# gk969/stm32-speech-recognition

Hardware: AMD Instinct MI355X
Metric: utterances/sec (256-frame, 100 templates) (higher is better)
Workload: dtype int32

## Files before the change

stm32_speech_recognition_amd/csrc/k_mfcc.hip:

```cpp
#include "sr_fft_dev.h"

#include <type_traits>

#ifndef SR_MEL_CHUNKED
#define SR_MEL_CHUNKED 1
#endif

namespace sr {

constexpr int kMfccWaves = 4;
constexpr int kFramesPerWave = 16, kFramesPerWaveMid = 4, kFramesPerWaveSmall = 1;
#ifndef SR_MAG_TAB_BINS
#define SR_MAG_TAB_BINS 8
#endif
constexpr int mfcc_tab_bins(int fpw) { return fpw == kFramesPerWave ? SR_MAG_TAB_BINS : 0; }
static_assert(SR_MAG_TAB_BINS == 0 || SR_MAG_TAB_BINS == 4 || SR_MAG_TAB_BINS == 8, "table bins per lane");
#ifndef SR_MFCC_PIPE
#define SR_MFCC_PIPE 1
#endif
#ifndef SR_MFCC_PIPE_PEEL
#define SR_MFCC_PIPE_PEEL 1
#endif
#ifndef SR_MFCC_PIPE_VMCNT
#define SR_MFCC_PIPE_VMCNT (SR_MFCC_PIPE_PEEL ? 3 : 0)
#endif
static_assert(SR_MFCC_PIPE_VMCNT == 0 || (SR_MFCC_PIPE_VMCNT == 3 && SR_MFCC_PIPE_PEEL), "younger loads counted by the wait");
constexpr bool mfcc_pipelined(int fpw) { return SR_MFCC_PIPE && mfcc_tab_bins(fpw) == 8; }
constexpr int kMelPad = kMel + 1;
__device__ __forceinline__ constexpr int mel_chunk_word(int j) { return 256 * ((j >> 2) & 1) + 4 * ((j >> 3) ^ (4 * ((j >> 2) & 1))) + (j & 3); }
constexpr int mfcc_wave_lds_words(int fpw) { return kXchgWords + fpw * kMelPad + 64; }

template <typename Base>
struct MfccTabArgs : Base {
    const uint16_t *mag_q;
    uint32_t mag_table_off;
};
template <typename Base>
constexpr int mfcc_feat_kind<MfccTabArgs<Base>> = mfcc_feat_kind<Base>;
template <typename Base>
static MfccTabArgs<Base> mfcc_tab_args(const Base &b, const MfccMagTab &tab)
{
    MfccTabArgs<Base> r;
    static_cast<Base &>(r) = b;
    r.mag_q = tab.mag_q;
    r.mag_table_off = tab.mag_table_off;
    return r;
}

template <int kFPW, typename Args = MfccTabArgs<MfccArgs>>
__global__ void __launch_bounds__(64 * kMfccWaves, 4) k_mfcc(const Args a)
{
    constexpr int kFeat = mfcc_feat_kind<Args>;
    constexpr uint32_t kFeatW = (kFeat == SR_FEAT_FFT || kFeat == SR_FEAT_MAG) ? kBins : kMel;
    constexpr int kWaveLdsWords = mfcc_wave_lds_words(kFPW);
    constexpr int kTabBins = mfcc_tab_bins(kFPW);
    constexpr bool kPipe = mfcc_pipelined(kFPW);
    extern __shared__ __attribute__((aligned(16))) uint32_t smem[];
    __shared__ uint32_t s_dctM[kCoef * kMelPad];
    __shared__ int s_dctS[kCoef * kMelPad];
    __shared__ u32x4 s_tw3[kTw3Row * 4], s_tw5[8 * 64];
    __shared__ u32x4 s_tm[4 * 64];
    const int lane = threadIdx.x & 63, w = __builtin_amdgcn_readfirstlane(threadIdx.x >> 6);
    uint32_t *buf = smem + w * kWaveLdsWords;
    uint32_t *xw = buf;
    uint32_t *powb = buf + kXchgWords, *moff = powb + kFPW * kMelPad;

    for (int i = threadIdx.x; i < kCoef * kMel; i += blockDim.x) {
        const int c = a.t.dct[i], o = (i / kMel) * kMelPad + i % kMel;
        s_dctM[o] = (uint32_t)(((c < 0 ? -c : c) * 262144 + 99) / 100);
        s_dctS[o] = (c > 0) - (c < 0);
    }
    __syncthreads();

    LaneTw tw;
    load_lane_tw(a.t, lane, tw);
    real_leg_tw(tw);
    if (w == 0 && lane < 4) {
        const uint32_t *f = &tw.s3[0][0][0];
#pragma unroll
        for (int c = 0; c < 8; c++) s_tw3[lane * kTw3Row + c] = u32x4{f[4 * c], f[4 * c + 1], f[4 * c + 2], f[4 * c + 3]};
    }
    if (w == 1 % kMfccWaves) store_tw32(s_tw5, lane, tw.s5);
#ifndef SR_INJECT_LDS_RACE
    if (w == 2 % kMfccWaves) {
#pragma unroll
        for (int c = 0; c < 2; c++) {
            s_tm[64 * c + lane] = *(const u32x4 *)(a.t.tri_even_m + 8 * lane + 4 * c);
            s_tm[64 * (c + 2) + lane] = *(const u32x4 *)(a.t.tri_odd_m + 8 * lane + 4 * c);
        }
    }
#endif
    __syncthreads();
#ifdef SR_INJECT_LDS_RACE
    if (w == 2 % kMfccWaves) {
#if SR_INJECT_LDS_RACE >= 2
        __builtin_amdgcn_s_sleep(127);
#endif
#pragma unroll
        for (int c = 0; c < 2; c++) {
            s_tm[64 * c + lane] = *(const u32x4 *)(a.t.tri_even_m + 8 * lane + 4 * c);
            s_tm[64 * (c + 2) + lane] = *(const u32x4 *)(a.t.tri_odd_m + 8 * lane + 4 * c);
        }
    }
#endif
    int hamm_m[3];
#pragma unroll
    for (int k = 0; k < 3; k++) hamm_m[k] = (lane + 64 * k < kFrameLen) ? hamm_fused_multiplier(a.t.hamm[lane + 64 * k]) : 0;
    int f_lo = 0, p_hi = 0, p_lo = 0, x_hi = 0, x_lo = 0;
    if (lane < kMel) {
        const int h = lane;
        f_lo = (h == 0) ? 0 : (int)a.t.tri_cen[h - 1];
        const int f_hi = (h == kMel - 1) ? kBins : (int)a.t.tri_cen[h + 1];
        const int ih = f_hi - 1, il = f_lo ? f_lo - 1 : 0, half = (h & 1) ? kBins : 0;
#if SR_MEL_CHUNKED
        p_hi = half + mel_chunk_word(ih), x_hi = (ih >> 3) > 0 ? (ih >> 3) - 1 : 0;
        p_lo = half + mel_chunk_word(il), x_lo = (il >> 3) > 0 ? (il >> 3) - 1 : 0;
#else
        p_hi = half + ih, x_hi = (ih >> 3) > 0 ? (ih >> 3) - 1 : 0;
        p_lo = half + il, x_lo = (il >> 3) > 0 ? (il >> 3) - 1 : 0;
#endif
    }
    const uint64_t mag_p = (uint64_t)a.mag_q;
    const u32x4 mag_rs = {(uint32_t)mag_p, (uint32_t)(mag_p >> 32) | (2u << 16), kMagTabEntries, 0x00027000u};
    const uint32_t tw_off = 32u * (uint32_t)lane;
#if SR_MEL_CHUNKED
    const int e_base = mel_chunk_word(lane);
    constexpr int kEs = 32, kEh = 128;
    const int c0 = mel_chunk_word(8 * lane), c1 = mel_chunk_word(8 * lane + 4);
#else
    const int e_base = lane;
    constexpr int kEs = 64, kEh = 256;
    const int c0 = 8 * lane, c1 = 8 * lane + 4;
#endif

    uint32_t item = blockIdx.x;
    uint32_t nx_nfrm = 0;
    int nx_mid = 0, nx_seg0 = 0;
    if (item < a.n_items) {
        const sr_vad_rec *rec = a.vad + item / a.tiles;
        nx_nfrm = rec->frm_num;
        nx_mid = (int)rec->atap.mid_val;
        nx_seg0 = rec->seg[0];
    }
    for (; item < a.n_items; item += gridDim.x) {
        const uint32_t b = item / a.tiles, tile = item - b * a.tiles;
        const uint32_t nfrm = nx_nfrm;
        const int mid = nx_mid, seg0 = nx_seg0;
        if (item + gridDim.x < a.n_items) {
            const sr_vad_rec *rec = a.vad + (item + gridDim.x) / a.tiles;
            nx_nfrm = rec->frm_num;
            nx_mid = (int)rec->atap.mid_val;
            nx_seg0 = rec->seg[0];
        }
        const uint16_t *row = a.pcm + (uint64_t)b * a.pcm_stride;
        int16_t *out = a.mfcc + (uint64_t)b * a.max_frames * kCoef;
        const uint32_t f0 = tile * (kMfccWaves * kFPW) + w * kFPW;
        uint32_t *frow = nullptr;
        if constexpr (kFeat != 0) frow = a.feat + (uint64_t)b * a.max_frames * kFeatW;
        uint32_t nf = 0;
        if (f0 < nfrm) nf = (nfrm - f0 < (uint32_t)kFPW) ? nfrm - f0 : (uint32_t)kFPW;

        uint32_t s_pp[3] = {0, 0, 0};
        if (nf) {
            const uint16_t *x = row + seg0 + (int)kHop * (int)f0;
#pragma unroll
            for (int k = 0; k < 3; k++) {
                const int i = lane + 64 * k;
                if (i < kFrameLen) s_pp[k] = *(const u32_align2 *)(x + i - 1);
            }
        }
        if constexpr (!kPipe)
        for (uint32_t fi = 0; fi < nf; fi++) {
#pragma unroll
            for (int k = 0; k < 3; k++) {
                const int i = lane + 64 * k;
                if (i < kFrameLen) k == 0 ? window_store<0>(xw, i, s_pp[k], mid, hamm_m[k]) : window_store<1>(xw, i, s_pp[k], mid, hamm_m[k]);
            }
            if (fi + 1 < nf) {
                const uint16_t *x = row + seg0 + (int)kHop * (int)(f0 + fi + 1);
#pragma unroll
                for (int k = 0; k < 3; k++) {
                    const int i = lane + 64 * k;
                    if (i < kFrameLen) s_pp[k] = *(const u32_align2 *)(x + i - 1);
                }
            }
            wave_sync();
            uint32_t v[4][4], u[4][4];
            fft_front_real160(xw, lane, tw, s_tw3, v);
            fft_exchange(buf, lane, v, u);
#pragma unroll
            for (int e4 = 0; e4 < 4; e4++) fft_pass4_dbl(u, e4, tw);
            wave_sync();
            uint32_t k5[4][4][2];
            load_tw32(s_tw5, lane, k5);
            uint32_t nn[8];
#pragma unroll
            for (int e3 = 0; e3 < 4; e3++) {
                bfly_pk_dbl<true, false, 0>(u[e3][0], u[e3][1], u[e3][2], u[e3][3], k5[e3][0][0], k5[e3][0][1], k5[e3][1][0],
                                            k5[e3][1][1], k5[e3][2][0], k5[e3][2][1], k5[e3][3][0], k5[e3][3][1]);
                if constexpr (kFeat == SR_FEAT_FFT) {
                    uint32_t *fr = frow + (f0 + fi) * kFeatW + lane + 64 * e3;
                    fr[0] = u[e3][0];
                    fr[256] = u[e3][1];
                }
                nn[2 * e3] = (uint32_t)sdot2z(u[e3][0], u[e3][0]);
                nn[2 * e3 + 1] = (uint32_t)sdot2z(u[e3][1], u[e3][1]);
            }
            const uint32_t nmax = max(max(max(max(nn[0], nn[1]), nn[2]), max(max(nn[3], nn[4]), nn[5])), max(nn[6], nn[7]));
#ifdef SR_TESTING
            const bool quiet = __builtin_expect(__builtin_amdgcn_ballot_w64(nmax > kMagSmallMax) == 0 && !a.mag_table_off, 1);
#else
            const bool quiet = __builtin_expect(__builtin_amdgcn_ballot_w64(nmax > kMagSmallMax) == 0, 1);
#endif
            u32x4 tw_e[2], tw_o[2];
            bool cheap = true;
            if (!quiet) {
#pragma unroll
                for (int c = 0; c < 2; c++) {
                    tw_e[c] = *(const u32x4 *)((const char *)a.t.tri_even32 + tw_off + 16 * c);
                    tw_o[c] = *(const u32x4 *)((const char *)a.t.tri_odd32 + tw_off + 16 * c);
                }
                cheap = __builtin_amdgcn_ballot_w64(nmax > a.mag_cheap_max) == 0;
            } else {
                asm volatile("" : "=v"(tw_e[0]), "=v"(tw_e[1]), "=v"(tw_o[0]), "=v"(tw_o[1]));
            }
            uint32_t *eb = buf + e_base;
            if (kTabBins > 0 && quiet) {
                uint32_t tq[8];
#pragma unroll
                for (int e3 = 0; e3 < 4; e3++) {
                    if constexpr (kTabBins == 8)
                        asm volatile("buffer_load_ushort %0, %1, %2, 0 idxen" : "=v"(tq[2 * e3]) : "v"(nn[2 * e3]), "s"(mag_rs));
                    asm volatile("buffer_load_ushort %0, %1, %2, 0 idxen" : "=v"(tq[2 * e3 + 1]) : "v"(nn[2 * e3 + 1]), "s"(mag_rs));
                }
                uint32_t q0s[4];
                if constexpr (kTabBins == 4) {
#pragma unroll
                    for (int e3 = 0; e3 < 4; e3++) q0s[e3] = cvt_u32(__builtin_amdgcn_sqrtf((float)(int)nn[2 * e3]) * 10.0f) << 2;
                }
                if constexpr (kTabBins == 8)
                    asm volatile("s_waitcnt vmcnt(0)" : "+v"(tq[0]), "+v"(tq[1]), "+v"(tq[2]), "+v"(tq[3]), "+v"(tq[4]), "+v"(tq[5]), "+v"(tq[6]), "+v"(tq[7]));
                else
                    asm volatile("s_waitcnt vmcnt(0)" : "+v"(tq[1]), "+v"(tq[3]), "+v"(tq[5]), "+v"(tq[7]));
#pragma unroll
                for (int e3 = 0; e3 < 4; e3++) {
                    uint32_t q0, q1 = tq[2 * e3 + 1];
                    if constexpr (kTabBins == 8) q0 = tq[2 * e3];
                    else q0 = q0s[e3];
                    if constexpr (kFeat == SR_FEAT_MAG) {
                        uint32_t *fr = frow + (f0 + fi) * kFeatW + lane + 64 * e3;
                        fr[0] = q0 >> 2;
                        fr[256] = q1 >> 2;
                    }
                    eb[kEs * e3] = umul24(q0, q0);
                    eb[kEs * e3 + kEh] = umul24(q1, q1);
                }
            } else if (cheap) {
#pragma unroll
                for (int e3 = 0; e3 < 4; e3++) {
                    const f32x2 m = f32x2{__builtin_amdgcn_sqrtf((float)(int)nn[2 * e3]), __builtin_amdgcn_sqrtf((float)(int)nn[2 * e3 + 1])} *
                                    f32x2{10.0f, 10.0f};
                    const uint32_t m0 = cvt_u32(m.x), m1 = cvt_u32(m.y);
                    if constexpr (kFeat == SR_FEAT_MAG) {
                        uint32_t *fr = frow + (f0 + fi) * kFeatW + lane + 64 * e3;
                        fr[0] = m0;
                        fr[256] = m1;
                    }
                    eb[kEs * e3] = umul24(m0, m0);
                    eb[kEs * e3 + kEh] = umul24(m1, m1);
                }
            } else {
#pragma unroll
                for (int e3 = 0; e3 < 4; e3++) {
                    const f32x2 m = sqrt_rn_int2(f32x2{(float)(int)nn[2 * e3], (float)(int)nn[2 * e3 + 1]}) * f32x2{10.0f, 10.0f};
                    const uint32_t m0 = cvt_u32(m.x), m1 = cvt_u32(m.y);
                    if constexpr (kFeat == SR_FEAT_MAG) {
                        uint32_t *fr = frow + (f0 + fi) * kFeatW + lane + 64 * e3;
                        fr[0] = m0;
                        fr[256] = m1;
                    }
                    eb[kEs * e3] = umul24(m0, m0);
                    eb[kEs * e3 + kEh] = umul24(m1, m1);
                }
            }
            wave_sync();
            uint32_t pe[8], po[8], xe, xo;
            {
                const uint4 q0 = *(const uint4 *)(buf + c0), q1 = *(const uint4 *)(buf + c1);
                const uint32_t e[8] = {q0.x, q0.y, q0.z, q0.w, q1.x, q1.y, q1.z, q1.w};
                uint32_t se = 0, so = 0;
                if (quiet) {
#pragma unroll
                    for (int c = 0; c < 2; c++) {
                        const u32x4 me = s_tm[64 * c + lane], mo = s_tm[64 * (c + 2) + lane];
#pragma unroll
                        for (int k = 0; k < 4; k++) {
                            const uint32_t es = kTabBins > 0 ? e[4 * c + k] : e[4 * c + k] << 4;
                            se += mel_term_fused(es, me[k]);
                            so += mel_term_fused(es, mo[k]);
                            pe[4 * c + k] = se;
                            po[4 * c + k] = so;
                        }
                    }
                } else {
#pragma unroll
                    for (int c = 0; c < 2; c++) {
#pragma unroll
                        for (int k = 0; k < 4; k++) {
                            se += e[4 * c + k] * tw_e[c][k] / 100u;
                            so += e[4 * c + k] * tw_o[c][k] / 100u;
                            pe[4 * c + k] = se;
                            po[4 * c + k] = so;
                        }
                    }
                }
                xe = wave_scan_incl(se);
                xo = wave_scan_incl(so);
            }
            *(uint4 *)(buf + c0) = make_uint4(pe[0], pe[1], pe[2], pe[3]);
            *(uint4 *)(buf + c1) = make_uint4(pe[4], pe[5], pe[6], pe[7]);
            *(uint4 *)(buf + kBins + c0) = make_uint4(po[0], po[1], po[2], po[3]);
            *(uint4 *)(buf + kBins + c1) = make_uint4(po[4], po[5], po[6], po[7]);
            buf[2 * kBins + lane] = xe;
            moff[lane] = xo;
            wave_sync();
            if (lane < kMel) {
                const uint32_t *X = (lane & 1) ? moff : buf + 2 * kBins;
                const uint32_t hi = buf[p_hi] + X[x_hi], lo = f_lo ? buf[p_lo] + X[x_lo] : 0u;
                powb[fi * kMelPad + lane] = hi - lo;
                if constexpr (kFeat == SR_FEAT_MEL) frow[(f0 + fi) * kFeatW + lane] = hi - lo;
            }
            wave_sync();
        } else {
            uint32_t mq[8] = {0, 0, 0, 0, 0, 0, 0, 0};
            bool pq = true;
            auto window = [&]() {
#pragma unroll
                for (int k = 0; k < 3; k++) {
                    const int i = lane + 64 * k;
                    if (i < kFrameLen) k == 0 ? window_store<0>(xw, i, s_pp[k], mid, hamm_m[k]) : window_store<1>(xw, i, s_pp[k], mid, hamm_m[k]);
                }
            };
            auto request = [&](uint32_t f) {
                const uint16_t *x = row + seg0 + (int)kHop * (int)(f0 + f);
#pragma unroll
                for (int k = 0; k < 3; k++) {
                    const int i = lane + 64 * k;
                    if (i < kFrameLen) s_pp[k] = *(const u32_align2 *)(x + i - 1);
                }
            };
            auto middle = [&](uint32_t fi, uint32_t (&v)[4][4], bool more) {
                uint32_t u[4][4];
                fft_exchange(buf, lane, v, u);
#pragma unroll
                for (int e4 = 0; e4 < 4; e4++) fft_pass4_dbl(u, e4, tw);
                wave_sync();
                uint32_t k5[4][4][2];
                load_tw32(s_tw5, lane, k5);
                uint32_t nn[8];
#pragma unroll
                for (int e3 = 0; e3 < 4; e3++) {
                    bfly_pk_dbl<true, false, 0>(u[e3][0], u[e3][1], u[e3][2], u[e3][3], k5[e3][0][0], k5[e3][0][1], k5[e3][1][0],
                                                k5[e3][1][1], k5[e3][2][0], k5[e3][2][1], k5[e3][3][0], k5[e3][3][1]);
                    if constexpr (kFeat == SR_FEAT_FFT) {
                        uint32_t *fr = frow + (f0 + fi) * kFeatW + lane + 64 * e3;
                        fr[0] = u[e3][0];
                        fr[256] = u[e3][1];
                    }
                    nn[2 * e3] = (uint32_t)sdot2z(u[e3][0], u[e3][0]);
                    nn[2 * e3 + 1] = (uint32_t)sdot2z(u[e3][1], u[e3][1]);
                }
                const uint32_t nmax = max(max(max(max(nn[0], nn[1]), nn[2]), max(max(nn[3], nn[4]), nn[5])), max(nn[6], nn[7]));
                if (more) {
                    wave_sync();
                    window();
                }
#ifdef SR_TESTING
                const bool quiet = __builtin_expect(__builtin_amdgcn_ballot_w64(nmax > kMagSmallMax) == 0 && !a.mag_table_off, 1);
#else
                const bool quiet = __builtin_expect(__builtin_amdgcn_ballot_w64(nmax > kMagSmallMax) == 0, 1);
#endif
                if (quiet) {
#pragma unroll
                    for (int k = 0; k < 8; k++) asm volatile("buffer_load_ushort %0, %1, %2, 0 idxen" : "=v"(mq[k]) : "v"(nn[k]), "s"(mag_rs));
                } else if (__builtin_amdgcn_ballot_w64(nmax > a.mag_cheap_max) == 0) {
#pragma unroll
                    for (int e3 = 0; e3 < 4; e3++) {
                        const f32x2 m = f32x2{__builtin_amdgcn_sqrtf((float)(int)nn[2 * e3]), __builtin_amdgcn_sqrtf((float)(int)nn[2 * e3 + 1])} *
                                        f32x2{10.0f, 10.0f};
                        mq[2 * e3] = cvt_u32(m.x);
                        mq[2 * e3 + 1] = cvt_u32(m.y);
                    }
                } else {
#pragma unroll
                    for (int e3 = 0; e3 < 4; e3++) {
                        const f32x2 m = sqrt_rn_int2(f32x2{(float)(int)nn[2 * e3], (float)(int)nn[2 * e3 + 1]}) * f32x2{10.0f, 10.0f};
                        mq[2 * e3] = cvt_u32(m.x);
                        mq[2 * e3 + 1] = cvt_u32(m.y);
                    }
                }
                pq = quiet;
                if (fi + 2 < nf) request(fi + 2);
            };
            auto back_end = [&](uint32_t r, auto young) {
                wave_sync();
                auto energies = [&]() {
                    uint32_t *eb = buf + e_base;
#pragma unroll
                    for (int e3 = 0; e3 < 4; e3++) {
                        const uint32_t q0 = mq[2 * e3], q1 = mq[2 * e3 + 1];
                        if constexpr (kFeat == SR_FEAT_MAG) {
                            uint32_t *fr = frow + (f0 + r) * kFeatW + lane + 64 * e3;
                            const uint32_t sh = pq ? 2u : 0u;
                            fr[0] = q0 >> sh;
                            fr[256] = q1 >> sh;
                        }
                        eb[kEs * e3] = umul24(q0, q0);
                        eb[kEs * e3 + kEh] = umul24(q1, q1);
                    }
                    wave_sync();
                };
                uint32_t pe[8], po[8], se = 0, so = 0;
                if (pq) {
                    if constexpr (decltype(young)::value)
                        asm volatile("s_waitcnt vmcnt(3)" : "+v"(mq[0]), "+v"(mq[1]), "+v"(mq[2]), "+v"(mq[3]), "+v"(mq[4]), "+v"(mq[5]), "+v"(mq[6]), "+v"(mq[7]));
                    else
                        asm volatile("s_waitcnt vmcnt(0)" : "+v"(mq[0]), "+v"(mq[1]), "+v"(mq[2]), "+v"(mq[3]), "+v"(mq[4]), "+v"(mq[5]), "+v"(mq[6]), "+v"(mq[7]));
                    energies();
                    const uint4 q0 = *(const uint4 *)(buf + c0), q1 = *(const uint4 *)(buf + c1);
                    const uint32_t e[8] = {q0.x, q0.y, q0.z, q0.w, q1.x, q1.y, q1.z, q1.w};
#pragma unroll
                    for (int c = 0; c < 2; c++) {
                        const u32x4 me = s_tm[64 * c + lane], mo = s_tm[64 * (c + 2) + lane];
#pragma unroll
                        for (int k = 0; k < 4; k++) {
                            se += mel_term_fused(e[4 * c + k], me[k]);
                            so += mel_term_fused(e[4 * c + k], mo[k]);
                            pe[4 * c + k] = se;
                            po[4 * c + k] = so;
                        }
                    }
                } else {
                    u32x4 tw_e[2], tw_o[2];
                    uint32_t off = tw_off;
                    asm("" : "+v"(off));
#pragma unroll
                    for (int c = 0; c < 2; c++) {
                        tw_e[c] = *(const u32x4 *)((const char *)a.t.tri_even32 + off + 16 * c);
                        tw_o[c] = *(const u32x4 *)((const char *)a.t.tri_odd32 + off + 16 * c);
                    }
                    energies();
                    const uint4 q0 = *(const uint4 *)(buf + c0), q1 = *(const uint4 *)(buf + c1);
                    const uint32_t e[8] = {q0.x, q0.y, q0.z, q0.w, q1.x, q1.y, q1.z, q1.w};
#pragma unroll
                    for (int c = 0; c < 2; c++) {
#pragma unroll
                        for (int k = 0; k < 4; k++) {
                            se += e[4 * c + k] * tw_e[c][k] / 100u;
                            so += e[4 * c + k] * tw_o[c][k] / 100u;
                            pe[4 * c + k] = se;
                            po[4 * c + k] = so;
                        }
                    }
                }
                const uint32_t xe = wave_scan_incl(se), xo = wave_scan_incl(so);
                *(uint4 *)(buf + c0) = make_uint4(pe[0], pe[1], pe[2], pe[3]);
                *(uint4 *)(buf + c1) = make_uint4(pe[4], pe[5], pe[6], pe[7]);
                *(uint4 *)(buf + kBins + c0) = make_uint4(po[0], po[1], po[2], po[3]);
                *(uint4 *)(buf + kBins + c1) = make_uint4(po[4], po[5], po[6], po[7]);
                buf[2 * kBins + lane] = xe;
                moff[lane] = xo;
                wave_sync();
                if (lane < kMel) {
                    const uint32_t *X = (lane & 1) ? moff : buf + 2 * kBins;
                    const uint32_t hi = buf[p_hi] + X[x_hi], lo = f_lo ? buf[p_lo] + X[x_lo] : 0u;
                    powb[r * kMelPad + lane] = hi - lo;
                    if constexpr (kFeat == SR_FEAT_MEL) frow[(f0 + r) * kFeatW + lane] = hi - lo;
                }
                wave_sync();
            };
            constexpr std::false_type kDrain{};
            if (nf) {
                window();
                if (nf > 1) request(1);
#if SR_MFCC_PIPE_PEEL
                constexpr std::integral_constant<bool, SR_MFCC_PIPE_VMCNT != 0> kSteady{};
                {
                    wave_sync();
                    uint32_t v[4][4];
                    fft_front_real160(xw, lane, tw, s_tw3, v);
                    middle(0, v, nf > 1);
                }
                for (uint32_t fi = 1; fi + 1 < nf; fi++) {
                    wave_sync();
                    uint32_t v[4][4];
                    fft_front_real160(xw, lane, tw, s_tw3, v);
                    back_end(fi - 1, kSteady);
                    middle(fi, v, true);
                }
                if (nf > 1) {
                    wave_sync();
                    uint32_t v[4][4];
                    fft_front_real160(xw, lane, tw, s_tw3, v);
                    back_end(nf - 2, kDrain);
                    middle(nf - 1, v, false);
                }
#else
                for (uint32_t fi = 0; fi < nf; fi++) {
                    wave_sync();
                    uint32_t v[4][4];
                    fft_front_real160(xw, lane, tw, s_tw3, v);
                    if (fi > 0) back_end(fi - 1, kDrain);
                    middle(fi, v, fi + 1 < nf);
                }
#endif
                back_end(nf - 1, kDrain);
            }
        }

        {
            constexpr int kLogRounds = (kFPW * kMelPad + 63) / 64;
            const uint32_t n_log = nf * kMelPad;
            uint32_t nv[kLogRounds], mv[kLogRounds];
            u32x2 tv[kLogRounds];
#pragma unroll
            for (int r = 0; r < kLogRounds; r++) {
                const uint32_t t = lane + 64u * r;
                nv[r] = powb[t];
                mv[r] = log100_est(nv[r]);
                tv[r] = *(const u32_pair_align4 *)((const char *)a.t.log_thr + 4u * mv[r]);
            }
#pragma unroll
            for (int r = 0; r < kLogRounds; r++) {
                const uint32_t t = lane + 64u * r;
                if (t < n_log) powb[t] = log100_fix(nv[r], mv[r], tv[r].x, tv[r].y) << 14;
            }
        }
        wave_sync();
        if constexpr (kFeat == SR_FEAT_LOGMEL) {
            uint32_t *fw = frow + f0 * kFeatW;
            for (uint32_t t = lane; t < nf * kFeatW; t += 64) {
                const uint32_t fi = t / kFeatW, h = t - fi * kFeatW;
                fw[t] = powb[fi * kMelPad + h] >> 14;
            }
        }
        {
            int16_t *out_w = out + (size_t)f0 * kCoef;
#pragma unroll
            for (uint32_t tl = lane; tl < (uint32_t)(kFPW * kCoef); tl += 64) {
                uint32_t t = tl;
                if constexpr (kPipe) asm volatile("" : "+v"(t));
                if (t < nf * kCoef) {
                    const uint32_t fi = umul24(t, 10923u) >> 17, h = t - umul24(fi, (uint32_t)kCoef);
                    const uint32_t *pw = powb + umul24(fi, (uint32_t)kMelPad), *dm = s_dctM + umul24(h, (uint32_t)kMelPad);
                    const int *ds = s_dctS + umul24(h, (uint32_t)kMelPad);
                    int acc = 0;
#pragma unroll
                    for (int i = 0; i < kMel; i++) acc = mad24((int)__umulhi(pw[i], dm[i]), ds[i], acc);
                    out_w[t] = (int16_t)acc;
                }
            }
        }
        wave_sync();
        {
            const uint32_t r0 = f0 + nf, r1 = (f0 + kFPW < a.max_frames) ? f0 + kFPW : a.max_frames;
            for (uint32_t t = r0 * kCoef + lane; t < r1 * kCoef && r0 < r1; t += 64) out[t] = 0;
        }
        if constexpr (kFeat != 0) {
            const uint32_t r0 = f0 + nf, r1 = (f0 + kFPW < a.max_frames) ? f0 + kFPW : a.max_frames;
            for (uint32_t t = r0 * kFeatW + lane; t < r1 * kFeatW && r0 < r1; t += 64) frow[t] = 0;
        }
    }
}

uint32_t mfcc_ext_frames_per_tile();
int mfcc_ext_occupancy(int *per_cu);
void launch_mfcc_ext(const MfccArgs &a, uint32_t grid, hipStream_t s);
void launch_mfcc_ext_features(const MfccArgs &a, int kind, uint32_t *feat, uint32_t grid, hipStream_t s);

uint32_t mfcc_frames_per_tile(uint32_t frame_len) { return frame_len == 320 ? mfcc_ext_frames_per_tile() : (uint32_t)(kMfccWaves * kFramesPerWave); }
uint32_t mfcc_frames_per_tile_small(uint32_t frame_len, uint32_t which)
{
    return frame_len == 320 ? mfcc_ext_frames_per_tile() : (uint32_t)(kMfccWaves * (which ? kFramesPerWaveSmall : kFramesPerWaveMid));
}

uint32_t mfcc_resident_workgroups(uint32_t frame_len)
{
    int dev = 0, n_cu = 0, per_cu = 0;
    if (hipGetDevice(&dev) != hipSuccess) return 0;
    if (hipDeviceGetAttribute(&n_cu, hipDeviceAttributeMultiprocessorCount, dev) != hipSuccess || n_cu < 1) return 0;
    int e;
    if (frame_len == 320)
        e = mfcc_ext_occupancy(&per_cu);
    else
// ... 73 lines not shown
```

stm32_speech_recognition_amd/csrc/sr_dev.h:

```cpp
#pragma once
#include <cstdlib>

#include "sr_device.h"
#include "sr_tables.h"

namespace sr {

typedef short short2v __attribute__((ext_vector_type(2)));
typedef uint32_t u32x2 __attribute__((ext_vector_type(2)));
typedef uint32_t u32x4 __attribute__((ext_vector_type(4)));

__device__ __forceinline__ int sdot2(uint32_t a, uint32_t b, int c)
{
    return __builtin_amdgcn_sdot2(__builtin_bit_cast(short2v, a), __builtin_bit_cast(short2v, b), c, false);
}
__device__ __forceinline__ int sext_lo(uint32_t w) { return (int)(short)(w & 0xFFFFu); }
__device__ __forceinline__ int sext_hi(uint32_t w) { return (int)w >> 16; }
__device__ __forceinline__ uint32_t pack16(int re, int im) { return ((uint32_t)re & 0xFFFFu) | ((uint32_t)im << 16); }

__device__ __forceinline__ int sdot2z(uint32_t a, uint32_t b)
{
    int r;
    asm("v_dot2_i32_i16 %0, %1, %2, 0" : "=v"(r) : "v"(a), "v"(b));
    return r;
// ... 40 lines not shown
__device__ __forceinline__ float sqrt_rn_int(float f)
{
    const float y = __builtin_amdgcn_rsqf(f);
    const float s0 = f * y, h = 0.5f * y;
    const float r = __builtin_fmaf(-s0, s0, f);
    return __builtin_fmaf(r, h, s0);
}

__device__ __forceinline__ uint32_t mag10_small(float f)
{
    uint32_t r;
    const float m = __builtin_amdgcn_sqrtf(f) * 10.0f;
    asm("v_cvt_u32_f32 %0, %1" : "=v"(r) : "v"(m));
    return r;
}

__device__ __forceinline__ uint32_t cvt_u32(float x)
{
    uint32_t r;
    asm("v_cvt_u32_f32 %0, %1" : "=v"(r) : "v"(x));
    return r;
}
typedef float f32x2 __attribute__((ext_vector_type(2)));
__device__ __forceinline__ f32x2 sqrt_rn_int2(f32x2 f)
{
    const f32x2 y = {__builtin_amdgcn_rsqf(f.x), __builtin_amdgcn_rsqf(f.y)};
    const f32x2 s0 = f * y, h = f32x2{0.5f, 0.5f} * y;
    const f32x2 r = __builtin_elementwise_fma(-s0, s0, f);
    return __builtin_elementwise_fma(r, h, s0);
}
typedef uint32_t u32_align2 __attribute__((aligned(2)));
typedef uint32_t u32x2_raw __attribute__((ext_vector_type(2)));
typedef u32x2_raw u32_pair_align4 __attribute__((aligned(4)));
typedef uint32_t u32x2_align2 __attribute__((ext_vector_type(2), aligned(2)));

typedef unsigned short u16x2 __attribute__((ext_vector_type(2)));
__device__ __forceinline__ uint32_t pk_add(uint32_t a, uint32_t b)
{
    return __builtin_bit_cast(uint32_t, (u16x2)(__builtin_bit_cast(u16x2, a) + __builtin_bit_cast(u16x2, b)));
}
__device__ __forceinline__ uint32_t pk_sub(uint32_t a, uint32_t b)
{
    return __builtin_bit_cast(uint32_t, (u16x2)(__builtin_bit_cast(u16x2, a) - __builtin_bit_cast(u16x2, b)));
}
__device__ __forceinline__ uint32_t pk_ashr(uint32_t a, int n)
{
    return __builtin_bit_cast(uint32_t, (short2v)(__builtin_bit_cast(short2v, a) >> (short2v){(short)n, (short)n}));
}
__device__ __forceinline__ uint32_t pk_lshr(uint32_t a, int n)
{
    return __builtin_bit_cast(uint32_t, (u16x2)(__builtin_bit_cast(u16x2, a) >> (u16x2){(unsigned short)n, (unsigned short)n}));
}
__device__ __forceinline__ uint32_t pk_mad(uint32_t a, uint32_t c, uint32_t b)
{
    return __builtin_bit_cast(uint32_t, (u16x2)(__builtin_bit_cast(u16x2, a) * __builtin_bit_cast(u16x2, c) +
                                                __builtin_bit_cast(u16x2, b)));
}
__device__ __forceinline__ uint32_t pk_mad_swap(uint32_t a, uint32_t c, uint32_t b)
{
    uint32_t r;
    asm("v_pk_mad_u16 %0, %1, %2, %3 op_sel:[1,0,0] op_sel_hi:[0,1,1]" : "=v"(r) : "v"(a), "s"(c), "v"(b));
    return r;
}
template <bool VC, int L1, int H1, bool SWAP = false>
__device__ __forceinline__ uint32_t pk_mad_sel(uint32_t a, uint32_t c, uint32_t b)
{
    uint32_t r;
    if constexpr (VC)
        asm("v_pk_mad_u16 %0, %1, %2, %3 op_sel:[%4,%5,0] op_sel_hi:[%6,%7,1]" : "=v"(r) : "v"(a), "v"(c), "v"(b), "n"(SWAP ? 1 : 0), "n"(L1), "n"(SWAP ? 0 : 1), "n"(H1));
    else
        asm("v_pk_mad_u16 %0, %1, %2, %3 op_sel:[%4,%5,0] op_sel_hi:[%6,%7,1]" : "=v"(r) : "v"(a), "s"(c), "v"(b), "n"(SWAP ? 1 : 0), "n"(L1), "n"(SWAP ? 0 : 1), "n"(H1));
    return r;
}
__device__ __forceinline__ uint32_t pk_mul_lo_lo(uint32_t a, uint32_t c)
{
    uint32_t r;
    asm("v_pk_mul_lo_u16 %0, %1, %2 op_sel:[0,0] op_sel_hi:[1,0]" : "=v"(r) : "v"(a), "v"(c));
    return r;
}
__device__ __forceinline__ uint32_t pk_mul_lo_dup(uint32_t a, uint32_t c)
{
    uint32_t r;
    asm("v_pk_mul_lo_u16 %0, %1, %2 op_sel_hi:[0,1]" : "=v"(r) : "v"(a), "s"(c));
    return r;
}
__device__ __forceinline__ uint32_t pk_hi16(int lo_src, int hi_src)
{
    return __builtin_amdgcn_perm((uint32_t)hi_src, (uint32_t)lo_src, 0x07060302u);
}
__device__ __forceinline__ uint32_t pk_s15(int lo_src, int hi_src)
{
    uint32_t r = (uint32_t)lo_src >> 15;
    asm("v_lshrrev_b32_sdwa %0, %1, %2 dst_sel:WORD_1 dst_unused:UNUSED_PRESERVE src0_sel:DWORD src1_sel:DWORD\n\ts_nop 0"
        : "+v"(r)
        : "v"(15), "v"(hi_src));
    return r;
}

__device__ __forceinline__ void wave_sync()
{
    __builtin_amdgcn_fence(__ATOMIC_RELEASE, "wavefront");
    __builtin_amdgcn_wave_barrier();
    __builtin_amdgcn_fence(__ATOMIC_ACQUIRE, "wavefront");
}

__device__ __forceinline__ uint32_t wave_sum(uint32_t v)
{
#pragma unroll
    for (int d = 32; d >= 1; d >>= 1) v += __shfl_xor(v, d, 64);
    return v;
}
__device__ __forceinline__ uint32_t wave_min_u32(uint32_t v)
{
#pragma unroll
    for (int d = 32; d >= 1; d >>= 1) {
        uint32_t o = __shfl_xor(v, d, 64);
        v = o < v ? o : v;
    }
    return v;
}
__device__ __forceinline__ uint32_t wave_max(uint32_t v)
{
#pragma unroll
    for (int d = 32; d >= 1; d >>= 1) {
        uint32_t o = __shfl_xor(v, d, 64);
        v = o > v ? o : v;
    }
    return v;
}

template <int CTRL, int ROW_MASK>
__device__ __forceinline__ uint32_t dpp_take(uint32_t v)
{
    return (uint32_t)__builtin_amdgcn_update_dpp(0, (int)v, CTRL, ROW_MASK, 0xF, false);
}
__device__ __forceinline__ uint32_t wave_scan_incl(uint32_t v)
{
    v += dpp_take<0x111, 0xF>(v);
    v += dpp_take<0x112, 0xF>(v);
    v += dpp_take<0x114, 0xF>(v);
    v += dpp_take<0x118, 0xF>(v);
    asm("s_nop 1\n\tv_add_u32_dpp %0, %0, %0 row_bcast:15 row_mask:0xa" : "+v"(v));
    asm("s_nop 1\n\tv_add_u32_dpp %0, %0, %0 row_bcast:31 row_mask:0xc" : "+v"(v));
    return v;
}

__device__ __forceinline__ uint32_t log100_est(uint32_t n)
{
    return (uint32_t)(int)__builtin_amdgcn_fmed3f(__log2f((float)n) * 69.31471806f, 1.0f, (float)(kLogMax - 1));
}
__device__ __forceinline__ uint32_t log100_fix(uint32_t n, uint32_t m, uint32_t t0, uint32_t t1)
{
    return (uint32_t)((int)m - (int)(n < t0) + (int)(n >= t1));
}
__device__ __forceinline__ uint32_t log100_u32(uint32_t n, const uint32_t *__restrict__ thr)
{
    const uint32_t m = log100_est(n);
    return log100_fix(n, m, thr[m], thr[m + 1]);
}

}
```

stm32_speech_recognition_amd/csrc/sr_fft_dev.h:

```cpp
#pragma once
#include <type_traits>

#include "sr_dev.h"

namespace sr {

__device__ __forceinline__ void cxmul(uint32_t y, uint32_t ka, uint32_t kb, int &re, int &im)
{
    re = sdot2z(y, ka);
    im = sdot2z(y, kb);
}

template <int S>
__device__ __forceinline__ void r4_combine(int &ar, int &ai, int &br, int &bi, int &cr, int &ci, int &dr, int &di)
{
    int tr = cr + dr, ti = ci + di;
    dr = cr - dr;
    di = ci - di;
    cr = tr;
    ci = ti;
    ar >>= 2;
    ai >>= 2;
    ar += br >> (2 + S);
    ai += bi >> (2 + S);
// ... 102 lines not shown
__device__ __forceinline__ void bfly_pk_dbl(uint32_t &x0, uint32_t &x1, uint32_t &x2, uint32_t &x3, uint32_t k1a,
                                            uint32_t k1b, uint32_t k2a, uint32_t k2b, uint32_t k3a, uint32_t k3b,
                                            uint32_t k3na, uint32_t k3nb, uint32_t mul = 0)
{
    int br, bi, cr, ci;
    cxmul(x2, k2a, k2b, cr, ci);
    cxmul(x1, k1a, k1b, br, bi);
    const int sr = sdot2a(x3, k3a, cr), si = sdot2a(x3, k3b, ci);
    const int tr = sdot2a(x3, k3na, cr), ti = sdot2a(x3, k3nb, ci);
    uint32_t a = pk_ashr(x0, 2);
    if (OUT == 1) a = pk_add(a, a);
    if (OUT == 2) a = pk_mul_lo_lo(a, mul);
    r4_packed_dbl<HALF, true, false, DBL_CD, OUT>(a, mul, br, bi, sr, si, tr, ti, x0, x1, x2, x3);
}

__device__ __forceinline__ uint32_t pk_neg(uint32_t w) { return pk_sub(0u, w); }

__device__ __forceinline__ void bfly(uint32_t &x0, uint32_t &x1, uint32_t &x2, uint32_t &x3, uint32_t k1a, uint32_t k1b,
                                     uint32_t k2a, uint32_t k2b, uint32_t k3a, uint32_t k3b)
{
    bfly_pk<false>(x0, x1, x2, x3, k1a, k1b, k2a, k2b, k3a, k3b, pk_neg(k3a), pk_neg(k3b));
}

__device__ __forceinline__ int rev2(int d) { return ((d & 1) << 1) | (d >> 1); }

__device__ __forceinline__ int xaddr(int j) { return j + ((j >> 6) << 2); }
constexpr int kXchgWords = 1024 + 4 * 16;

struct LaneTw {
    uint32_t s2[2][2];
    uint32_t s3[4][4][2];
    uint32_t s4[4][2];
    uint32_t s5[4][4][2];
};

__device__ __forceinline__ void load_tw3(const DevTables &t, int base, int b, uint32_t (&k)[3][2])
{
    const int e = base + 3 * b;
    k[0][0] = t.tw_a[e + 2];
    k[0][1] = t.tw_b[e + 2];
    k[1][0] = t.tw_a[e + 1];
    k[1][1] = t.tw_b[e + 1];
    k[2][0] = t.tw_a[e + 0];
    k[2][1] = t.tw_b[e + 0];
}

__device__ __forceinline__ void load_tw4(const DevTables &t, int base, int b, uint32_t (&k)[4][2])
{
    uint32_t k3[3][2];
    load_tw3(t, base, b, k3);
#pragma unroll
    for (int e = 0; e < 3; e++) {
        k[e][0] = k3[e][0];
        k[e][1] = k3[e][1];
    }
    k[3][0] = pk_sub(0u, k3[2][0]);
    k[3][1] = pk_sub(0u, k3[2][1]);
}

__device__ __forceinline__ void load_lane_tw(const DevTables &t, int lane, LaneTw &tw)
{
    const int d0 = lane & 3;
    {
        uint32_t k[3][2];
        load_tw3(t, 0, d0, k);
        tw.s2[0][0] = k[0][0];
        tw.s2[0][1] = k[0][1];
        tw.s2[1][0] = k[1][0];
        tw.s2[1][1] = k[1][1];
    }
#pragma unroll
    for (int d1 = 0; d1 < 4; d1++) load_tw4(t, 12, d0 + 4 * d1, tw.s3[d1]);
    load_tw4(t, 60, lane, tw.s4);
#pragma unroll
    for (int d3 = 0; d3 < 4; d3++) load_tw4(t, 252, lane + 64 * d3, tw.s5[d3]);
}

__device__ __forceinline__ void store_tw32(u32x4 *lds, int lane, const uint32_t (&k)[4][4][2])
{
    const uint32_t *f = &k[0][0][0];
#pragma unroll
    for (int c = 0; c < 8; c++) lds[c * 64 + lane] = u32x4{f[4 * c], f[4 * c + 1], f[4 * c + 2], f[4 * c + 3]};
}
__device__ __forceinline__ void load_tw32(const u32x4 *lds, int lane, uint32_t (&k)[4][4][2])
{
    uint32_t *f = &k[0][0][0];
#pragma unroll
    for (int c = 0; c < 8; c++) {
        const u32x4 q = lds[c * 64 + lane];
        f[4 * c] = q.x;
        f[4 * c + 1] = q.y;
        f[4 * c + 2] = q.z;
        f[4 * c + 3] = q.w;
    }
}
constexpr int kTw3Row = 9;
__device__ __forceinline__ void load_tw32_d0(const u32x4 *lds, int d0, uint32_t (&k)[4][4][2])
{
    uint32_t *f = &k[0][0][0];
#pragma unroll
    for (int c = 0; c < 8; c++) {
        const u32x4 q = lds[d0 * kTw3Row + c];
        f[4 * c] = q.x;
        f[4 * c + 1] = q.y;
        f[4 * c + 2] = q.z;
        f[4 * c + 3] = q.w;
    }
}

constexpr uint32_t kPkOneTwo = 0x00020001u;
template <int K>
__device__ __forceinline__ void window_store(uint32_t *xw, int i, uint32_t prev_cur, int mid, int hm)
{
    if (K == 0) {
        xw[i] = pk_mul_lo_dup(window_sample<4>(prev_cur, mid, hm), kPkOneTwo);
    } else {
        const uint32_t y = window_sample<2>(prev_cur, mid, hm);
        xw[i] = y;
        ((uint16_t *)(xw + i))[1] = (uint16_t)y;
    }
}
__device__ __forceinline__ void real_leg_tw(LaneTw &tw)
{
#pragma unroll
    for (int l = 0; l < 2; l++)
#pragma unroll
        for (int w = 0; w < 2; w++) tw.s2[l][w] = __builtin_amdgcn_perm(0u, tw.s2[l][w], 0x01000100u);
}
__device__ __forceinline__ void fft_front_real160(const uint32_t *xw, int lane, const LaneTw &tw, const u32x4 *tw3_lds,
                                                  uint32_t (&v)[4][4])
{
    const int d3 = (lane >> 2) & 3, d4 = lane >> 4;
    const int base = rev2(d4) + 4 * rev2(d3);
    uint32_t y[10];
    y[0] = *(const uint16_t *)(xw + base);
#pragma unroll
    for (int m = 1; m < 4; m++) y[m] = ((const uint16_t *)(xw + base + 16 * m))[1];
#pragma unroll
    for (int m = 4; m < 10; m++) y[m] = xw[base + 16 * m];
#pragma unroll
    for (int m = 0; m < 4; m++) asm("" : "+v"(y[m]));
#pragma unroll
    for (int d2 = 0; d2 < 4; d2++) {
        const int r2 = ((d2 & 1) << 1) | (d2 >> 1);
        uint32_t x0 = y[r2];
        uint32_t x2 = y[4 + r2];
        uint32_t x1 = (d2 == 0) ? y[8] : (d2 == 2) ? y[9] : 0u;
        uint32_t x3 = 0u;
        int cr, ci;
        cxmul(x2, tw.s2[1][0], tw.s2[1][1], cr, ci);
        (void)x3;
        if (d2 == 0) {
            int br, bi;
            cxmul(x1, tw.s2[0][0], tw.s2[0][1], br, bi);
            r4_packed_dbl<false, true, true, true, 0>(x0, 0u, br, bi, cr, ci, cr, ci, v[0][d2], v[1][d2], v[2][d2], v[3][d2]);
        } else if (d2 == 2) {
            int br, bi;
            cxmul(x1, tw.s2[0][0], tw.s2[0][1], br, bi);
            r4_packed_dbl<false, true, true, true, 1>(x0, 0u, br, bi, cr, ci, cr, ci, v[0][d2], v[1][d2], v[2][d2], v[3][d2]);
        } else {
            r4_packed_dbl<false, false, true, true, 1>(x0, 0u, 0, 0, cr, ci, cr, ci, v[0][d2], v[1][d2], v[2][d2], v[3][d2]);
        }
    }
    uint32_t k3[4][4][2];
    load_tw32_d0(tw3_lds, lane & 3, k3);
    const uint32_t mul = d3 ? kPkTwo : kPkPlusMinus;
#pragma unroll
    for (int d1 = 0; d1 < 4; d1++)
        bfly_pk_dbl<false, true, 2>(v[d1][0], v[d1][1], v[d1][2], v[d1][3], k3[d1][0][0], k3[d1][0][1], k3[d1][1][0], k3[d1][1][1],
                                    k3[d1][2][0], k3[d1][2][1], k3[d1][3][0], k3[d1][3][1], mul);
}

__device__ __forceinline__ void fft_exchange(uint32_t *buf, int lane, const uint32_t (&v)[4][4], uint32_t (&u)[4][4])
{
    const int d0 = lane & 3, d3 = (lane >> 2) & 3, d4 = lane >> 4;
    const int jw = d0 + 64 * d3 + 256 * d4;
#pragma unroll
    for (int d1 = 0; d1 < 4; d1++)
#pragma unroll
        for (int d2 = 0; d2 < 4; d2++) buf[xaddr(jw + 4 * d1 + 16 * d2)] = v[d1][d2];
    wave_sync();
#pragma unroll
    for (int e3 = 0; e3 < 4; e3++)
#pragma unroll
        for (int e4 = 0; e4 < 4; e4++) u[e3][e4] = buf[xaddr(lane + 64 * e3 + 256 * e4)];
}

__device__ __forceinline__ void fft_pass4_dbl(uint32_t (&u)[4][4], int e4, const LaneTw &tw)
{
    if (e4 == 1)
        bfly_pk_dbl<false, true, 1>(u[0][e4], u[1][e4], u[2][e4], u[3][e4], tw.s4[0][0], tw.s4[0][1], tw.s4[1][0], tw.s4[1][1],
                                    tw.s4[2][0], tw.s4[2][1], tw.s4[3][0], tw.s4[3][1]);
    else
        bfly_pk_dbl<false, true, 0>(u[0][e4], u[1][e4], u[2][e4], u[3][e4], tw.s4[0][0], tw.s4[0][1], tw.s4[1][0], tw.s4[1][1],
                                    tw.s4[2][0], tw.s4[2][1], tw.s4[3][0], tw.s4[3][1]);
}

__device__ __forceinline__ int bitrev8(int v) { return (int)(__brev((uint32_t)v) >> 24); }

__device__ inline void fft_full_wave(const uint32_t *__restrict__ in, uint32_t *__restrict__ out, uint32_t *buf, int lane,
                              const DevTables &t)
{
    for (int m = 0; m < 4; m++) {
        const int idx = lane + 64 * m, r = bitrev8(idx);
        const uint32_t wa = in[r], wc = in[r + 256], wb = in[r + 512], wd = in[r + 768];
        int ar = sext_lo(wa), ai = sext_hi(wa), br = sext_lo(wb), bi = sext_hi(wb);
        int cr = sext_lo(wc), ci = sext_hi(wc), dr = sext_lo(wd), di = sext_hi(wd);
        r4_combine<0>(ar, ai, br, bi, cr, ci, dr, di);
        buf[xaddr(4 * idx + 0)] = pack16(ar, ai);
        buf[xaddr(4 * idx + 1)] = pack16(br, bi);
        buf[xaddr(4 * idx + 2)] = pack16(cr, ci);
        buf[xaddr(4 * idx + 3)] = pack16(di, dr);
    }
    wave_sync();
    LaneTw tw;
    load_lane_tw(t, lane, tw);
    uint32_t k2[3][2];
    load_tw3(t, 0, lane & 3, k2);
    const int d0 = lane & 3, d3 = (lane >> 2) & 3, d4 = lane >> 4;
    uint32_t v[4][4], u[4][4];
#pragma unroll
    for (int d1 = 0; d1 < 4; d1++)
#pragma unroll
        for (int d2 = 0; d2 < 4; d2++) v[d1][d2] = buf[xaddr(d0 + 4 * d1 + 16 * d2 + 64 * d3 + 256 * d4)];
    wave_sync();
#pragma unroll
    for (int d2 = 0; d2 < 4; d2++)
        bfly(v[0][d2], v[1][d2], v[2][d2], v[3][d2], k2[0][0], k2[0][1], k2[1][0], k2[1][1], k2[2][0], k2[2][1]);
#pragma unroll
    for (int d1 = 0; d1 < 4; d1++)
        bfly(v[d1][0], v[d1][1], v[d1][2], v[d1][3], tw.s3[d1][0][0], tw.s3[d1][0][1], tw.s3[d1][1][0],
             tw.s3[d1][1][1], tw.s3[d1][2][0], tw.s3[d1][2][1]);
    fft_exchange(buf, lane, v, u);
#pragma unroll
    for (int e4 = 0; e4 < 4; e4++)
        bfly(u[0][e4], u[1][e4], u[2][e4], u[3][e4], tw.s4[0][0], tw.s4[0][1], tw.s4[1][0], tw.s4[1][1], tw.s4[2][0],
             tw.s4[2][1]);
#pragma unroll
    for (int e3 = 0; e3 < 4; e3++) {
        bfly(u[e3][0], u[e3][1], u[e3][2], u[e3][3], tw.s5[e3][0][0], tw.s5[e3][0][1], tw.s5[e3][1][0],
             tw.s5[e3][1][1], tw.s5[e3][2][0], tw.s5[e3][2][1]);
#pragma unroll
        for (int e4 = 0; e4 < 4; e4++) out[lane + 64 * e3 + 256 * e4] = u[e3][e4];
    }
}

}
```

Baseline: 3.363 million.

## Issue twiddle and next-frame gather LDS reads ahead of FFT compute in MFCC

Splits the FFT front end into a gather step and a compute step, and splits the twiddle loads so the first rows are issued before the butterfly passes. Sched barriers pin those early reads in place. In the pipelined path, the next frame's windowed samples are gathered right after the window store, so the LDS latency overlaps other work. The packed 1/2 scaling moves from a scalar constant to a per-lane vector multiplier, which lets the gather use plain word loads instead of 16-bit half loads. The cost is higher register pressure and a more rigid schedule, and an ISA analysis script is added to check how much latency each wait hides.

```diff
diff --git a/profiles/isa_wait_cover.py b/profiles/isa_wait_cover.py
--- /dev/null
+++ b/profiles/isa_wait_cover.py
@@ -0,0 +1,73 @@
+import re
+import sys
+
+STORE = re.compile(r"ds_(write|add|or|and|min|max|sub|xor|inc|dec)")
+
+
+def kernel_blocks(path, kern):
+    lines = open(path).read().split("\n")
+    start = next(i for i, l in enumerate(lines) if re.match(r"^_ZN2sr\d+" + kern + r"[EI]", l))
+    blocks, cur = {"entry": []}, "entry"
+    for l in lines[start + 1:]:
+        if l.strip().startswith("s_endpgm"):
+            break
+        m = re.match(r"^(\.LBB\d+_\d+):", l) or re.match(r"^; (%bb\.\d+):", l)
+        if m:
+            cur = m.group(1)
+            blocks[cur] = []
+            continue
+        m = re.match(r"^\s+([a-z_0-9]+)\b(.*)", l)
+        if m:
+            blocks[cur].append((m.group(1), m.group(2).split(";")[0]))
+    return blocks
+
+
+def wait_cover(ins):
+    valu, queue, rows, trip = 0, [], [], 0
+    for i, (blk, op, args) in enumerate(ins + ins):
+        second = i >= len(ins)
+        if op.startswith("v_"):
+            valu += 1
+        elif op.startswith("ds_"):
+            queue.append(("store" if STORE.match(op) and "_rtn" not in op else "read", valu, op, blk, second))
+            trip += bool(rows) and rows[-1][6] == trip
+        elif op.startswith(("s_load", "s_buffer_load")):
+            queue.append(("smem", valu, op, blk, second))
+        elif op == "s_waitcnt":
+            m = re.search(r"lgkmcnt\((\d+)\)", args)
+            if not m:
+                continue
+            n = int(m.group(1))
+            gone, queue = queue[:max(0, len(queue) - n)], queue[max(0, len(queue) - n):]
+            if not second:
+                continue
+            reads = [g for g in gone if g[0] == "read"]
+            if not reads:
+                rows.append((blk, n, None, "stores only" if gone else "nothing outstanding", 0, len(gone), trip))
+            else:
+                where = reads[0][3] + ("" if reads[0][4] else ", previous iteration")
+                rows.append((blk, n, valu - reads[0][1], "%s (%s)" % (reads[0][2], where), len(reads), len(gone), trip))
+    return rows, valu // 2
+
+
+def main():
+    path, kern, names = sys.argv[1], sys.argv[2], sys.argv[3:]
+    blocks = kernel_blocks(path, kern)
+    ins = [(n, op, args) for n in names for op, args in blocks[n]]
+    rows, valu = wait_cover(ins)
+    print("block        wait          cover  retires reads / all   oldest read waited for")
+    for blk, n, cover, what, nr, na, _ in rows:
+        c = "    -" if cover is None else "%5d" % cover
+        print(f"{blk:12s} lgkmcnt({n:<2d})  {c}  {nr:7d} / {na:<3d}         {what}")
+    cov = [r[2] for r in rows if r[2] is not None]
+    first = {}
+    for r in rows:
+        if r[2] is not None:
+            first.setdefault(r[6], r[2])
+    smem = sum(op.startswith(("s_load", "s_buffer_load")) for _, op, _ in ins)
+    print("waits for reads: %d, with cover <= 2: %d; round trips: %d, exposed (first wait's cover <= 2): %d; VALU on the path: %d%s"
+          % (len(cov), sum(c <= 2 for c in cov), len(first), sum(c <= 2 for c in first.values()), valu, "; SCALAR LOADS ON THE PATH: %d" % smem if smem else ""))
+
+
+if __name__ == "__main__":
+    main()
diff --git a/stm32_speech_recognition_amd/csrc/k_mfcc.hip b/stm32_speech_recognition_amd/csrc/k_mfcc.hip
--- a/stm32_speech_recognition_amd/csrc/k_mfcc.hip
+++ b/stm32_speech_recognition_amd/csrc/k_mfcc.hip
@@ -26,6 +26,11 @@
 #endif
 static_assert(SR_MFCC_PIPE_VMCNT == 0 || (SR_MFCC_PIPE_VMCNT == 3 && SR_MFCC_PIPE_PEEL), "younger loads counted by the wait");
 constexpr bool mfcc_pipelined(int fpw) { return SR_MFCC_PIPE && mfcc_tab_bins(fpw) == 8; }
+#ifndef SR_MFCC_READ_AHEAD
+#define SR_MFCC_READ_AHEAD 7
+#endif
+constexpr int kTw5Ahead = (SR_MFCC_READ_AHEAD & 1) ? 2 : 0, kTw3Ahead = (SR_MFCC_READ_AHEAD & 2) ? 2 : 0;
+constexpr bool kGatherAhead = (SR_MFCC_READ_AHEAD & 4) != 0;
 constexpr int kMelPad = kMel + 1;
 __device__ __forceinline__ constexpr int mel_chunk_word(int j) { return 256 * ((j >> 2) & 1) + 4 * ((j >> 3) ^ (4 * ((j >> 2) & 1))) + (j & 3); }
 constexpr int mfcc_wave_lds_words(int fpw) { return kXchgWords + fpw * kMelPad + 64; }
@@ -106,6 +111,8 @@
     int hamm_m[3];
 #pragma unroll
     for (int k = 0; k < 3; k++) hamm_m[k] = (lane + 64 * k < kFrameLen) ? hamm_fused_multiplier(a.t.hamm[lane + 64 * k]) : 0;
+    uint32_t a_mul = a_leg_mul(lane);
+    asm volatile("" : "+v"(a_mul));
     int f_lo = 0, p_hi = 0, p_lo = 0, x_hi = 0, x_lo = 0;
     if (lane < kMel) {
         const int h = lane;
@@ -174,7 +181,7 @@
 #pragma unroll
             for (int k = 0; k < 3; k++) {
                 const int i = lane + 64 * k;
-                if (i < kFrameLen) k == 0 ? window_store<0>(xw, i, s_pp[k], mid, hamm_m[k]) : window_store<1>(xw, i, s_pp[k], mid, hamm_m[k]);
+                if (i < kFrameLen) k == 0 ? window_store<0>(xw, i, s_pp[k], mid, hamm_m[k], a_mul) : window_store<1>(xw, i, s_pp[k], mid, hamm_m[k], 0u);
             }
             if (fi + 1 < nf) {
                 const uint16_t *x = row + seg0 + (int)kHop * (int)(f0 + fi + 1);
@@ -186,13 +193,9 @@
             }
             wave_sync();
             uint32_t v[4][4], u[4][4];
-            fft_front_real160(xw, lane, tw, s_tw3, v);
-            fft_exchange(buf, lane, v, u);
-#pragma unroll
-            for (int e4 = 0; e4 < 4; e4++) fft_pass4_dbl(u, e4, tw);
-            wave_sync();
+            fft_front_real160<kTw3Ahead>(xw, lane, tw, s_tw3, v);
             uint32_t k5[4][4][2];
-            load_tw32(s_tw5, lane, k5);
+            fft_exchange_pass4<kTw5Ahead>(buf, lane, tw, s_tw5, v, u, k5);
             uint32_t nn[8];
 #pragma unroll
             for (int e3 = 0; e3 < 4; e3++) {
@@ -332,13 +335,13 @@
             }
             wave_sync();
         } else {
-            uint32_t mq[8] = {0, 0, 0, 0, 0, 0, 0, 0};
+            uint32_t mq[8] = {0, 0, 0, 0, 0, 0, 0, 0}, y[10];
             bool pq = true;
             auto window = [&]() {
 #pragma unroll
                 for (int k = 0; k < 3; k++) {
                     const int i = lane + 64 * k;
-                    if (i < kFrameLen) k == 0 ? window_store<0>(xw, i, s_pp[k], mid, hamm_m[k]) : window_store<1>(xw, i, s_pp[k], mid, hamm_m[k]);
+                    if (i < kFrameLen) k == 0 ? window_store<0>(xw, i, s_pp[k], mid, hamm_m[k], a_mul) : window_store<1>(xw, i, s_pp[k], mid, hamm_m[k], 0u);
                 }
             };
             auto request = [&](uint32_t f) {
@@ -350,13 +353,8 @@
                 }
             };
             auto middle = [&](uint32_t fi, uint32_t (&v)[4][4], bool more) {
-                uint32_t u[4][4];
-                fft_exchange(buf, lane, v, u);
-#pragma unroll
-                for (int e4 = 0; e4 < 4; e4++) fft_pass4_dbl(u, e4, tw);
-                wave_sync();
-                uint32_t k5[4][4][2];
-                load_tw32(s_tw5, lane, k5);
+                uint32_t u[4][4], k5[4][4][2];
+                fft_exchange_pass4<kTw5Ahead>(buf, lane, tw, s_tw5, v, u, k5);
                 uint32_t nn[8];
 #pragma unroll
                 for (int e3 = 0; e3 < 4; e3++) {
@@ -374,6 +372,13 @@
                 if (more) {
                     wave_sync();
                     window();
+                    if constexpr (kGatherAhead) {
+                        wave_sync();
+                        fft_gather_real160(xw, lane, y);
+                        __builtin_amdgcn_sched_barrier(0);
+                    }
+                } else {
+                    asm volatile("" ::"v"(s_pp[0]), "v"(s_pp[1]), "v"(s_pp[2]));
                 }
 #ifdef SR_TESTING
                 const bool quiet = __builtin_expect(__builtin_amdgcn_ballot_w64(nmax > kMagSmallMax) == 0 && !a.mag_table_off, 1);
@@ -480,6 +485,10 @@
                 wave_sync();
             };
             constexpr std::false_type kDrain{};
+            auto front = [&](uint32_t (&v)[4][4], auto carried) {
+                if constexpr (!(decltype(carried)::value && kGatherAhead)) fft_gather_real160(xw, lane, y);
+                fft_pass23_real160<kTw3Ahead>(y, lane, tw, s_tw3, v);
+            };
             if (nf) {
                 window();
                 if (nf > 1) request(1);
@@ -488,20 +497,20 @@
                 {
                     wave_sync();
                     uint32_t v[4][4];
-                    fft_front_real160(xw, lane, tw, s_tw3, v);
+                    front(v, std::false_type{});
                     middle(0, v, nf > 1);
                 }
                 for (uint32_t fi = 1; fi + 1 < nf; fi++) {
                     wave_sync();
                     uint32_t v[4][4];
-                    fft_front_real160(xw, lane, tw, s_tw3, v);
+                    front(v, std::true_type{});
                     back_end(fi - 1, kSteady);
                     middle(fi, v, true);
                 }
                 if (nf > 1) {
                     wave_sync();
                     uint32_t v[4][4];
-                    fft_front_real160(xw, lane, tw, s_tw3, v);
+                    front(v, std::true_type{});
                     back_end(nf - 2, kDrain);
                     middle(nf - 1, v, false);
                 }
@@ -509,7 +518,8 @@
                 for (uint32_t fi = 0; fi < nf; fi++) {
                     wave_sync();
                     uint32_t v[4][4];
-                    fft_front_real160(xw, lane, tw, s_tw3, v);
+                    if (fi == 0) front(v, std::false_type{});
+                    else front(v, std::true_type{});
                     if (fi > 0) back_end(fi - 1, kDrain);
                     middle(fi, v, fi + 1 < nf);
                 }
diff --git a/stm32_speech_recognition_amd/csrc/sr_dev.h b/stm32_speech_recognition_amd/csrc/sr_dev.h
--- a/stm32_speech_recognition_amd/csrc/sr_dev.h
+++ b/stm32_speech_recognition_amd/csrc/sr_dev.h
@@ -146,6 +146,12 @@
 {
     uint32_t r;
     asm("v_pk_mul_lo_u16 %0, %1, %2 op_sel_hi:[0,1]" : "=v"(r) : "v"(a), "s"(c));
+    return r;
+}
+__device__ __forceinline__ uint32_t pk_mul_lo_dup_v(uint32_t a, uint32_t c)
+{
+    uint32_t r;
+    asm("v_pk_mul_lo_u16 %0, %1, %2 op_sel_hi:[0,1]" : "=v"(r) : "v"(a), "v"(c));
     return r;
 }
 __device__ __forceinline__ uint32_t pk_hi16(int lo_src, int hi_src)
diff --git a/stm32_speech_recognition_amd/csrc/sr_fft_dev.h b/stm32_speech_recognition_amd/csrc/sr_fft_dev.h
--- a/stm32_speech_recognition_amd/csrc/sr_fft_dev.h
+++ b/stm32_speech_recognition_amd/csrc/sr_fft_dev.h
@@ -208,38 +208,29 @@
 #pragma unroll
     for (int c = 0; c < 8; c++) lds[c * 64 + lane] = u32x4{f[4 * c], f[4 * c + 1], f[4 * c + 2], f[4 * c + 3]};
 }
-__device__ __forceinline__ void load_tw32(const u32x4 *lds, int lane, uint32_t (&k)[4][4][2])
+template <int C0, int C1, int STRIDE>
+__device__ __forceinline__ void load_tw32_part(const u32x4 *p, uint32_t (&k)[4][4][2])
 {
     uint32_t *f = &k[0][0][0];
 #pragma unroll
-    for (int c = 0; c < 8; c++) {
-        const u32x4 q = lds[c * 64 + lane];
+    for (int c = C0; c < C1; c++) {
+        const u32x4 q = p[c * STRIDE];
         f[4 * c] = q.x;
         f[4 * c + 1] = q.y;
         f[4 * c + 2] = q.z;
         f[4 * c + 3] = q.w;
     }
 }
+__device__ __forceinline__ void load_tw32(const u32x4 *lds, int lane, uint32_t (&k)[4][4][2]) { load_tw32_part<0, 8, 64>(lds + lane, k); }
 constexpr int kTw3Row = 9;
-__device__ __forceinline__ void load_tw32_d0(const u32x4 *lds, int d0, uint32_t (&k)[4][4][2])
-{
-    uint32_t *f = &k[0][0][0];
-#pragma unroll
-    for (int c = 0; c < 8; c++) {
-        const u32x4 q = lds[d0 * kTw3Row + c];
-        f[4 * c] = q.x;
-        f[4 * c + 1] = q.y;
-        f[4 * c + 2] = q.z;
-        f[4 * c + 3] = q.w;
-    }
-}
-
-constexpr uint32_t kPkOneTwo = 0x00020001u;
+__device__ __forceinline__ void load_tw32_d0(const u32x4 *lds, int d0, uint32_t (&k)[4][4][2]) { load_tw32_part<0, 8, 1>(lds + d0 * kTw3Row, k); }
+
+__device__ __forceinline__ uint32_t a_leg_mul(int lane) { return lane < 16 ? 1u : 2u; }
 template <int K>
-__device__ __forceinline__ void window_store(uint32_t *xw, int i, uint32_t prev_cur, int mid, int hm)
+__device__ __forceinline__ void window_store(uint32_t *xw, int i, uint32_t prev_cur, int mid, int hm, uint32_t amul)
 {
     if (K == 0) {
-        xw[i] = pk_mul_lo_dup(window_sample<4>(prev_cur, mid, hm), kPkOneTwo);
+        xw[i] = pk_mul_lo_dup_v(window_sample<4>(prev_cur, mid, hm), amul);
     } else {
         const uint32_t y = window_sample<2>(prev_cur, mid, hm);
         xw[i] = y;
@@ -253,19 +244,24 @@
 #pragma unroll
         for (int w = 0; w < 2; w++) tw.s2[l][w] = __builtin_amdgcn_perm(0u, tw.s2[l][w], 0x01000100u);
 }
-__device__ __forceinline__ void fft_front_real160(const uint32_t *xw, int lane, const LaneTw &tw, const u32x4 *tw3_lds,
-                                                  uint32_t (&v)[4][4])
+__device__ __forceinline__ void fft_gather_real160(const uint32_t *xw, int lane, uint32_t (&y)[10])
 {
     const int d3 = (lane >> 2) & 3, d4 = lane >> 4;
     const int base = rev2(d4) + 4 * rev2(d3);
-    uint32_t y[10];
-    y[0] = *(const uint16_t *)(xw + base);
-#pragma unroll
-    for (int m = 1; m < 4; m++) y[m] = ((const uint16_t *)(xw + base + 16 * m))[1];
-#pragma unroll
-    for (int m = 4; m < 10; m++) y[m] = xw[base + 16 * m];
-#pragma unroll
-    for (int m = 0; m < 4; m++) asm("" : "+v"(y[m]));
+#pragma unroll
+    for (int m = 0; m < 10; m++) y[m] = xw[base + 16 * m];
+}
+template <int kAhead>
+__device__ __forceinline__ void fft_pass23_real160(const uint32_t (&y)[10], int lane, const LaneTw &tw, const u32x4 *tw3_lds,
+                                                   uint32_t (&v)[4][4])
+{
+    const int d3 = (lane >> 2) & 3;
+    const u32x4 *row3 = tw3_lds + (lane & 3) * kTw3Row;
+    uint32_t k3[4][4][2];
+    if constexpr (kAhead > 0) {
+        load_tw32_part<0, kAhead, 1>(row3, k3);
+        __builtin_amdgcn_sched_barrier(0);
+    }
 #pragma unroll
     for (int d2 = 0; d2 < 4; d2++) {
         const int r2 = ((d2 & 1) << 1) | (d2 >> 1);
@@ -288,13 +284,20 @@
             r4_packed_dbl<false, false, true, true, 1>(x0, 0u, 0, 0, cr, ci, cr, ci, v[0][d2], v[1][d2], v[2][d2], v[3][d2]);
         }
     }
-    uint32_t k3[4][4][2];
-    load_tw32_d0(tw3_lds, lane & 3, k3);
+    load_tw32_part<kAhead, 8, 1>(row3, k3);
     const uint32_t mul = d3 ? kPkTwo : kPkPlusMinus;
 #pragma unroll
     for (int d1 = 0; d1 < 4; d1++)
         bfly_pk_dbl<false, true, 2>(v[d1][0], v[d1][1], v[d1][2], v[d1][3], k3[d1][0][0], k3[d1][0][1], k3[d1][1][0], k3[d1][1][1],
                                     k3[d1][2][0], k3[d1][2][1], k3[d1][3][0], k3[d1][3][1], mul);
+}
+template <int kAhead = 0>
+__device__ __forceinline__ void fft_front_real160(const uint32_t *xw, int lane, const LaneTw &tw, const u32x4 *tw3_lds,
+                                                  uint32_t (&v)[4][4])
+{
+    uint32_t y[10];
+    fft_gather_real160(xw, lane, y);
+    fft_pass23_real160<kAhead>(y, lane, tw, tw3_lds, v);
 }
 
 __device__ __forceinline__ void fft_exchange(uint32_t *buf, int lane, const uint32_t (&v)[4][4], uint32_t (&u)[4][4])
@@ -320,6 +323,21 @@
     else
         bfly_pk_dbl<false, true, 0>(u[0][e4], u[1][e4], u[2][e4], u[3][e4], tw.s4[0][0], tw.s4[0][1], tw.s4[1][0], tw.s4[1][1],
                                     tw.s4[2][0], tw.s4[2][1], tw.s4[3][0], tw.s4[3][1]);
+}
+
+template <int kAhead>
+__device__ __forceinline__ void fft_exchange_pass4(uint32_t *buf, int lane, const LaneTw &tw, const u32x4 *tw5_lds,
+                                                   const uint32_t (&v)[4][4], uint32_t (&u)[4][4], uint32_t (&k5)[4][4][2])
+{
+    fft_exchange(buf, lane, v, u);
+    if constexpr (kAhead > 0) {
+        load_tw32_part<0, kAhead, 64>(tw5_lds + lane, k5);
+        __builtin_amdgcn_sched_barrier(0);
+    }
+#pragma unroll
+    for (int e4 = 0; e4 < 4; e4++) fft_pass4_dbl(u, e4, tw);
+    wave_sync();
+    load_tw32_part<kAhead, 8, 64>(tw5_lds + lane, k5);
 }
 
 __device__ __forceinline__ int bitrev8(int v) { return (int)(__brev((uint32_t)v) >> 24); }
```

Result: no change. 3.355 million (-0.2%).
